# elastic-ai/elastic-gpu-agent

Hardware: AMD Instinct MI355X
Metric: fractional pods/GPU + p50 Allocate() RPC latency at 1/2/4/8 MI355X (higher is better)
Workload: dtype n/a; 1 GPU; model=gpushare-device-plugin, scenario=mixed, pods_per_gpu=16, backend=amdsmi, mem_unit_mib=1, global_batch=16, seq_len=0, parallelism=1 agent x 1 GPUs (1 load ranks)

## Files before the change

### elastic_gpu_agent_amd/isolation/__init__.py

```python
from __future__ import annotations

import json
import os
import threading
from typing import Dict, List, Optional, Tuple

from .. import consts
from ..types import GPUDevice
from .cumask import mask_hex, mask_words_from_cus, parse_mask_hex

try:
    from .._fastwire import atomic_write as _native_atomic_write
except ImportError:
    _native_atomic_write = None

AUX_MASK_PREFIX = "mask/"

_PRIORITY_RANK = {"low": 0, "normal": 1, "high": 2}


def priority_rank(priority: Optional[str]) -> int:
    return _PRIORITY_RANK.get(priority or "normal", 1)


class _Alloc:
    __slots__ = ("gpu", "cus", "rank", "orig_n_cus")

    def __init__(self, gpu: int, cus: set, rank: int, orig_n_cus: int):
        self.gpu = gpu
        self.cus = cus
        self.rank = rank
        self.orig_n_cus = orig_n_cus


class CUMaskAllocator:

    def __init__(self, storage, devices: List[GPUDevice], on_remask=None):
        self._storage = storage
        self._devices = {d.index: d for d in devices}
        self._lock = threading.Lock()
        self.on_remask = on_remask
        self._used: Dict[int, set] = {}
        self._by_hash: Dict[str, _Alloc] = {}
        for key, val in storage.aux_items(AUX_MASK_PREFIX):
            rec = json.loads(val)
            cus = self._mask_cus(rec["cu_mask"])
            gpu = rec.get("gpu_index")
            a = _Alloc(gpu, cus, priority_rank(rec.get("priority")),
                       rec.get("orig_cu_count", len(cus)))
            self._by_hash[key[len(AUX_MASK_PREFIX):]] = a
            self._used.setdefault(gpu, set()).update(cus)

    @staticmethod
    def _mask_cus(hexmask: str) -> set:
        cus = set()
        for w_i, w in enumerate(parse_mask_hex(hexmask)):
            for b in range(32):
                if w >> b & 1:
                    cus.add(w_i * 32 + b)
        return cus

    def _live_cus(self, gpu_index: int) -> set:
        return self._used.setdefault(gpu_index, set())

    def _free_pairs_by_xcd(self, gpu_index: int, total: int, xcds: int) -> List[List[int]]:
        per_xcd = total // xcds
# ... 11 lines not shown

    @staticmethod
    def _take_round_robin(free_by_xcd: List[List[int]], want: int,
                          taken: List[int]) -> None:
        while len(taken) < want and any(free_by_xcd):
            progress = False
            for free in free_by_xcd:
                if len(taken) >= want:
                    break
                if free:
                    taken.append(free.pop(0))
                    progress = True
            if not progress:
                break

    def _persist(self, alloc_hash: str, a: _Alloc, total: int, percent: int) -> Tuple[str, int]:
        cus = sorted(a.cus)
        words = mask_words_from_cus(cus, total)
        hexmask = mask_hex(words)
        rank_name = {0: "low", 1: "normal", 2: "high"}[a.rank]
        self._storage.aux_set(
            AUX_MASK_PREFIX + alloc_hash,
            json.dumps(
                {
                    "gpu_index": a.gpu,
                    "cu_mask": hexmask,
                    "cu_count": len(cus),
                    "percent": percent,
                    "priority": rank_name,
                    "orig_cu_count": a.orig_n_cus,
                }
            ),
        )
        return hexmask, len(cus)

    def _remask_victim(self, victim_hash: str, a: _Alloc, total: int) -> None:
        raw = self._storage.aux_get(AUX_MASK_PREFIX + victim_hash)
        percent = json.loads(raw).get("percent", 0) if raw else 0
        hexmask, n_cus = self._persist(victim_hash, a, total, percent)
        if self.on_remask is not None:
            try:
                self.on_remask(victim_hash, hexmask, n_cus)
            except Exception:
                pass

    def _reclaim_locked(self, gpu_index: int, need_pairs: int, my_rank: int,
                        total: int) -> List[int]:
        victims = sorted(
            (
# ... 50 lines not shown
            if want_pairs <= 0:
                continue
            free_by_xcd = self._free_pairs_by_xcd(gpu_index, total, xcds)
            taken: List[int] = []
            self._take_round_robin(free_by_xcd, want_pairs, taken)
            if not taken:
                return
            for cu0 in taken:
                a.cus.add(cu0)
                a.cus.add(cu0 + 1)
                used.add(cu0)
                used.add(cu0 + 1)
            self._remask_victim(h, a, total)

    def allocate(self, alloc_hash: str, gpu_index: int, percent: int,
                 priority: Optional[str] = None) -> Tuple[str, int]:
        dev = self._devices.get(gpu_index)
        total = dev.cu_count if dev else consts.GFX950_CU_COUNT
        xcds = dev.xcd_count if dev else consts.GFX950_XCD_COUNT
        per_xcd = total // xcds
        from .cumask import cu_count_for_percent

        n = cu_count_for_percent(percent, total)
        pairs_per_xcd = per_xcd // 2
        rank = priority_rank(priority)
        with self._lock:
            old = self._by_hash.pop(alloc_hash, None)
            if old is not None:
                still = set()
                for a in self._by_hash.values():
                    if a.gpu == old.gpu:
                        still |= a.cus
                self._used.setdefault(old.gpu, set()).difference_update(old.cus - still)
            used = self._live_cus(gpu_index)
            want = (n + 1) // 2
            taken: List[int] = []
            self._take_round_robin(
                self._free_pairs_by_xcd(gpu_index, total, xcds), want, taken)
            if len(taken) < want and rank > 0:
                taken.extend(self._reclaim_locked(
                    gpu_index, want - len(taken), rank, total))
            if len(taken) < want:
                pair_max_rank: Dict[int, int] = {}
                for a in self._by_hash.values():
                    if a.gpu != gpu_index:
                        continue
                    for cu in a.cus:
                        cu0 = cu - (cu % 2)
                        if a.rank > pair_max_rank.get(cu0, -1):
                            pair_max_rank[cu0] = a.rank
                candidates = []
                for p in range(pairs_per_xcd):
                    for xcd in range(xcds):
                        cu0 = xcd * per_xcd + 2 * p
                        if cu0 not in taken:
                            candidates.append(cu0)
                candidates.sort(key=lambda cu0: pair_max_rank.get(cu0, -1) > rank)
                taken.extend(candidates[: want - len(taken)])
            cus: List[int] = []
            for cu0 in taken[:want]:
                cus.extend((cu0, cu0 + 1))
            a = _Alloc(gpu_index, set(cus), rank, len(cus))
            hexmask, n_eff = self._persist(alloc_hash, a, total, percent)
            self._by_hash[alloc_hash] = a
            used.update(a.cus)
        return hexmask, n_eff

    def _release_cached(self, alloc_hash: str) -> Optional[int]:
        entry = self._by_hash.pop(alloc_hash, None)
        if entry is None:
            return None
        used = self._used.setdefault(entry.gpu, set())
        still = set()
        for a in self._by_hash.values():
            if a.gpu == entry.gpu:
                still |= a.cus
        used.difference_update(entry.cus - still)
        return entry.gpu

    def _dev_geometry(self, gpu_index: int) -> Tuple[int, int]:
        dev = self._devices.get(gpu_index)
        total = dev.cu_count if dev else consts.GFX950_CU_COUNT
        xcds = dev.xcd_count if dev else consts.GFX950_XCD_COUNT
        return total, xcds

    def release(self, alloc_hash: str) -> None:
        with self._lock:
            gpu = self._release_cached(alloc_hash)
            if gpu is not None:
                self._expand_shrunk_locked(gpu, *self._dev_geometry(gpu))
        self._storage.aux_delete(AUX_MASK_PREFIX + alloc_hash)

    def release_many(self, hashes) -> None:
        hashes = list(hashes)
        with self._lock:
            gpus = {self._release_cached(h) for h in hashes}
            for gpu in gpus:
                if gpu is not None:
                    self._expand_shrunk_locked(gpu, *self._dev_geometry(gpu))
        self._storage.aux_delete_many(AUX_MASK_PREFIX + h for h in hashes)

    def get(self, alloc_hash: str) -> Optional[dict]:
        raw = self._storage.aux_get(AUX_MASK_PREFIX + alloc_hash)
        return json.loads(raw) if raw else None


class _TxnAux:

    def __init__(self, conn):
        self._conn = conn

    def aux_items(self, prefix: str = "") -> list:
        return self._conn.execute(
            "SELECT key, val FROM aux WHERE key LIKE ?", (prefix + "%",)
# ... 46 lines not shown
    def _base(self):
        ver = self._aux.aux_get(self.VER_KEY)
        if self._cached_base is None or ver != self._cached_ver or ver is None:
            self._cached_base = CUMaskAllocator(self._aux, self._devices,
                                                on_remask=self.on_remask)
        return self._cached_base

    def _bump(self) -> None:
        import uuid

        self._cached_ver = uuid.uuid4().hex
        self._aux.aux_set(self.VER_KEY, self._cached_ver)

    def _txn(self):
        class _Txn:
            def __init__(s, conn):
                s.conn = conn

            def __enter__(s):
                import fcntl

                fcntl.flock(s.fd, fcntl.LOCK_EX)
                s.conn.execute("BEGIN IMMEDIATE")
                return s

            def __exit__(s, et, ev, tb):
                import fcntl

                try:
                    if et is None:
                        try:
                            s.conn.execute("COMMIT")
                        except Exception:
                            try:
                                s.conn.execute("ROLLBACK")
                            except Exception:
                                pass
                            raise
                    else:
                        try:
                            s.conn.execute("ROLLBACK")
                        except Exception:
                            pass
                finally:
                    fcntl.flock(s.fd, fcntl.LOCK_UN)
                return False

        t = _Txn(self._conn)
        t.fd = self._flock_fd
        return t

    def allocate(self, alloc_hash: str, gpu_index: int, percent: int,
                 priority: Optional[str] = None) -> Tuple[str, int]:
        with self._local, self._txn():
            out = self._base().allocate(alloc_hash, gpu_index, percent,
                                        priority=priority)
            self._bump()
            return out

    def release(self, alloc_hash: str) -> None:
        with self._local, self._txn():
            self._base().release(alloc_hash)
            self._bump()
# ... 113 lines not shown
```

### elastic_gpu_agent_amd/native/build.py

```python
from __future__ import annotations

import os
import subprocess
import sys
import sysconfig

ROCM = os.environ.get("ROCM_PATH", "/opt/rocm")
HERE = os.path.dirname(os.path.abspath(__file__))
PKG = os.path.dirname(HERE)
REPO = os.path.dirname(PKG)


def _run(cmd):
    print("+", " ".join(cmd), flush=True)
    subprocess.check_call(cmd)


def _newer(target: str, *sources: str) -> bool:
    if not os.path.exists(target):
        return False
    t = os.path.getmtime(target)
    return all(os.path.getmtime(s) <= t for s in sources)


# ... 10 lines not shown
    if not force and _newer(out, src):
        return out
    _run(
        ["g++", "-O2", "-std=c++17", "-shared", "-fPIC", src]
        + pybind_includes()
        + [f"-I{ROCM}/include", f"-L{ROCM}/lib", "-lamd_smi",
           f"-Wl,-rpath,{ROCM}/lib", "-o", out]
    )
    return out


def build_fastwire(force=False):
    src = os.path.join(HERE, "fastwire.cpp")
    ext = sysconfig.get_config_var("EXT_SUFFIX")
    out = os.path.join(PKG, f"_fastwire{ext}")
    headers = [os.path.join(HERE, h) for h in ("wirecore.h", "idruns.h", "hashmemo.h", "bindfx.h")]
    if not force and _newer(out, src, *headers):
        return out
    _run(
        ["g++", "-O2", "-std=c++17", "-shared", "-fPIC", src]
        + pybind_includes()
        + ["-o", out, "-lcrypto"]
    )
    return out


def build_etransport(force=False):
    src = os.path.join(HERE, "etransport.cpp")
    tables = os.path.join(HERE, "hpack_tables.h")
    gen = os.path.join(HERE, "gen_hpack_tables.py")
    if not os.path.exists(tables) or os.path.getmtime(tables) < os.path.getmtime(gen):
# ... 70 lines not shown
```

### elastic_gpu_agent_amd/native/build_fuzz.py

```python
from __future__ import annotations

import os
import subprocess
import sys

HERE = os.path.dirname(os.path.abspath(__file__))
REPO = os.path.dirname(os.path.dirname(HERE))
CLANGXX = os.environ.get(
    "EGPU_FUZZ_CLANGXX", "/opt/rocm/lib/llvm/bin/clang++")


def build(out=None):
    out = out or os.path.join(REPO, "bin", "egpu-fuzz")
    os.makedirs(os.path.dirname(out), exist_ok=True)
    cmd = [
        CLANGXX, "-O1", "-g", "-std=c++17",
        "-fsanitize=fuzzer,address",
        os.path.join(HERE, "fuzz_targets.cpp"),
        os.path.join(HERE, "devfilter.cpp"),
        "-I", HERE, "-o", out,
    ]
    print("+", " ".join(cmd), flush=True)
    subprocess.check_call(cmd)
    return out
# ... 60 lines not shown
def build_h2frame_selftest(out=None):
    out = out or os.path.join(REPO, "bin", "egpu-h2frame-selftest")
    return build_selftest(out, "h2frame_selftest.cpp")


def build_hash_memo_selftest(out=None):
    out = out or os.path.join(REPO, "bin", "egpu-hash-memo-selftest")
    return build_selftest(out, "hash_memo_selftest.cpp")


def build_bindfx_selftest(out=None):
    out = out or os.path.join(REPO, "bin", "egpu-bindfx-selftest")
    return build_selftest(out, "bindfx_selftest.cpp")


if __name__ == "__main__":
    if "--selftest" in sys.argv:
        rc = subprocess.call([build_selftest()])
        rc = rc or subprocess.call([build_stride_selftest()])
        rc = rc or subprocess.call([build_runs_selftest()])
        rc = rc or subprocess.call([build_ref_selftest()])
        rc = rc or subprocess.call([build_mx_ref_selftest()])
        rc = rc or subprocess.call([build_h2frame_selftest()])
        rc = rc or subprocess.call([build_hash_memo_selftest()])
        sys.exit(rc or subprocess.call([build_bindfx_selftest()]))
    binary = build()
    if "--replay" in sys.argv:
        sys.exit(replay(binary))
    if "--run" in sys.argv:
        secs = int(sys.argv[sys.argv.index("--run") + 1])
        sys.exit(run(binary, secs))
```

### elastic_gpu_agent_amd/native/fastwire.cpp

```cpp

#include <pybind11/pybind11.h>
#include <pybind11/stl.h>

#include <openssl/evp.h>

#include <algorithm>
#include <cerrno>
#include <cstdint>
#include <stdexcept>
#include <string>
#include <utility>
#include <vector>

#include "bindfx.h"
#include "wirecore.h"

namespace py = pybind11;

namespace {

using wirecore::DigestOut;
using wirecore::DigestScratch;
using wirecore::Reader;
using wirecore::ScratchGuard;
using wirecore::Span;
using wirecore::span_less;
using wirecore::spans_of;

py::list decode_string_list(py::bytes data) {
// ... 522 lines not shown
    bindfx::atomic_write(path, buf, (size_t)len);
  } catch (const bindfx::SysError& e) {
    raise_oserror(e);
  }
}

void unlink_many(const std::vector<std::string>& paths) {
  try {
    py::gil_scoped_release rel;
    bindfx::unlink_many(paths);
  } catch (const bindfx::SysError& e) {
    raise_oserror(e);
  }
}

}

PYBIND11_MODULE(_fastwire, m) {
  m.doc() = "wire-format accelerators for large fake-device ID sets";
  m.def("decode_string_list", &decode_string_list);
  m.def("decode_nested_string_lists", &decode_nested_string_lists);
  m.def("encode_device_list", &encode_device_list);
  m.def("encode_string_list", &encode_string_list);
  m.def("encode_nested_string_lists", &encode_nested_string_lists);
  m.def("encode_allocate_response", &encode_allocate_response);
  m.def("digest_allocate_request", &digest_allocate_request);
  m.def("decode_prestart_digest", &decode_prestart_digest);
  m.def("decode_prestart_digest2", &decode_prestart_digest2);
  m.def("decode_prestart_digest3", &decode_prestart_digest3);
  m.def("ids_to_runs", &ids_to_runs);
  m.def("expand_runs", &expand_runs);
  m.def("preferred_digest", &preferred_digest);
  m.def("podresources_digest", &podresources_digest);
  m.def("preferred_extract", &preferred_extract);
  m.def("hash_memo_configure", &hash_memo_configure, py::arg("entries"));
  m.def("hash_memo_stats", &hash_memo_stats);
  m.attr("HASH_MEMO_ENTRIES") = (long long)wirecore::kMemoEntries;
  m.attr("HASH_MEMO_MAX_KEY") = (long long)wirecore::kMemoMaxKey;
  m.def("make_links", &make_links, py::arg("pairs"));
  m.def("atomic_write", &atomic_write, py::arg("path"), py::arg("data"));
  m.def("unlink_many", &unlink_many, py::arg("paths"));
}
```

### elastic_gpu_agent_amd/plugins/gpushare.py

```python
from __future__ import annotations

import logging
import math
import threading
from typing import List

from .. import consts, topology
from ..kube.client import NotFound
from ..types import Device
from .config import GPUPluginConfig

log = logging.getLogger(__name__)


class GPUSharePluginBase:

    resource_name: str = ""

    def __init__(self, config: GPUPluginConfig):
        self.cfg = config
        self._devices_lock = threading.Lock()
        self._refresh = threading.Event()

    def fake_device_ids_for_gpu(self, gpu) -> List[str]:
# ... 211 lines not shown
            return self._fail(
                context, f"pod {pc.pod()} lacks {consts.ELASTIC_GPU_ASSUMED_ANNOTATION}=true"
            )
        raw = pod.container_gpu_indexes(pc.container)
        if raw is None:
            return self._fail(
                context,
                f"pod {pc.pod()} lacks annotation for container {pc.container}",
            )
        try:
            indexes = [int(x) for x in raw.split(",") if x != ""]
        except ValueError:
            return self._fail(context, f"bad GPU index annotation {raw!r}")
        created: List[str] = []
        try:
            self._bind(device, indexes, created, pod)
            pi = self.cfg.storage.load_or_create(pc.namespace, pc.name)
            pi.container_device_map[pc.container] = device
            self.cfg.storage.save(pi)
        except Exception as e:
            for alloc_id in created:
                self.cfg.operator.delete(-1, alloc_id)
            if self.cfg.cumask is not None:
                try:
                    self.cfg.cumask.release(device.hash)
                except Exception:
                    pass
            if self.cfg.limits is not None:
                self.cfg.limits.delete(device.hash)
            self._emit_event(pc, "EgpuBindFailed", f"bind {device.hash}: {e}")
            return self._fail(context, f"bind {device.hash}: {e}")
        return {}

    def _bind(self, device: Device, indexes: List[int], created: List[str],
# ... 60 lines not shown
        return resp

    def _bind(self, device: Device, indexes: List[int], created: List[str],
              pod=None):
        n_links = self.links_for(device.n_ids)
        if len(indexes) != n_links:
            raise ValueError(
                f"annotation has {len(indexes)} GPU indexes, expected {n_links}"
            )
        for i, idx in enumerate(indexes):
            alloc_id = f"{device.hash}-{i}"
            self.cfg.operator.create(idx, alloc_id)
            created.append(alloc_id)
        percent = device.n_ids
        priority = pod.qos_class() if pod is not None else None
        if percent < consts.GPU_PERCENT_EACH_CARD and self.cfg.cumask and self.cfg.limits:
            mask_hex, n_cus = self.cfg.cumask.allocate(
                device.hash, indexes[0], percent, priority=priority)
            self.cfg.limits.finalize(
                device.hash,
                gpu_indexes=indexes,
                devices=self.cfg.operator.devices(),
                cu_mask=mask_hex,
                cu_count=n_cus,
                priority=priority,
            )
        elif self.cfg.limits:
            self.cfg.limits.finalize(
                device.hash, gpu_indexes=indexes, devices=self.cfg.operator.devices(),
                priority=priority,
            )

    def _locator(self):
        return self.cfg.core_locator


class GPUShareMemoryPlugin(GPUSharePluginBase):

    resource_name = consts.RESOURCE_GPU_MEMORY

    def fake_device_ids_for_gpu(self, gpu) -> List[str]:
        unit = self.cfg.options.mem_unit_mib
        count = gpu.memory_mib // unit
        return [f"{gpu.index}-{slot:06d}" for slot in range(count)]

    def _allocate_one(self, alloc_hash: str, n_units: int) -> dict:
# ... 35 lines not shown
```

### elastic_gpu_agent_amd/storage/__init__.py

```python
from __future__ import annotations

import fcntl
import os
import sqlite3
import threading
from typing import Callable, Optional

from ..types import PodInfo


class NotFoundError(KeyError):
    pass


class Storage:

    def __init__(self, db_path: str, record_format: str = "runs"):
        if record_format not in ("runs", "list"):
            raise ValueError(f"record format {record_format!r}: want runs or list")
        self._record_format = record_format
        db_dir = os.path.dirname(os.path.abspath(db_path))
        os.makedirs(db_dir, exist_ok=True)
        self._path = db_path
        self._lock = threading.Lock()
# ... 102 lines not shown
        done.wait()
        if res:
            raise res[0]

    SUMMARY_PREFIX = "podsum/"

    @staticmethod
    def _summary(pod_info: PodInfo) -> str:
        import json as _json

        return _json.dumps({
            c: {"h": d.hash, "n": d.n_ids, "r": d.resource_name}
            for c, d in pod_info.container_device_map.items()
        }, separators=(",", ":"))

    def save(self, pod_info: PodInfo) -> None:
        self._submit([
            ("INSERT INTO pods(key, val) VALUES(?, ?) "
             "ON CONFLICT(key) DO UPDATE SET val=excluded.val",
             (pod_info.key(), pod_info.stored_val()
              if self._record_format == "runs" else pod_info.val())),
            ("INSERT INTO aux(key, val) VALUES(?, ?) "
             "ON CONFLICT(key) DO UPDATE SET val=excluded.val",
             (self.SUMMARY_PREFIX + pod_info.key(), self._summary(pod_info))),
        ])

    def rewrite_as_lists(self) -> int:
        with self._lock:
            rows = self._conn.execute(
                "SELECT key, val FROM pods WHERE instr(val, ?) > 0", (b'"Runs":',)
            ).fetchall()
        n = 0
        for key, val in rows:
            literal = PodInfo.from_raw(key, val).val()
            if literal != bytes(val):
                self._submit([("UPDATE pods SET val=? WHERE key=? AND val=?",
                               (literal, key, val))])
                n += 1
        return n

# ... 151 lines not shown
```

Measured before the change: 2918 pod-allocation-cycles/s.

## Move CU-mask occupancy to native bitset allocator and batch mask rows into pod save

Adds a C++ CUOccupancy class that tracks per-GPU CU occupancy as bitsets and handles placement, reclaim and release, used by default when _fastwire is built. The pure-Python set-based path is kept as a fallback. Mask rows can now be deferred and written in the same storage transaction as the pod record, which removes a separate aux write per allocation. The trade-off is a larger native surface, and the native policy has to match the Python placement semantics.

```diff
diff --git a/elastic_gpu_agent_amd/isolation/__init__.py b/elastic_gpu_agent_amd/isolation/__init__.py
--- a/elastic_gpu_agent_amd/isolation/__init__.py
+++ b/elastic_gpu_agent_amd/isolation/__init__.py
@@ -13,6 +13,11 @@
     from .._fastwire import atomic_write as _native_atomic_write
 except ImportError:
     _native_atomic_write = None
+
+try:
+    from .._fastwire import CUOccupancy as _NativeOccupancy
+except ImportError:
+    _NativeOccupancy = None
 
 AUX_MASK_PREFIX = "mask/"
 
@@ -35,21 +40,44 @@
 
 class CUMaskAllocator:
 
-    def __init__(self, storage, devices: List[GPUDevice], on_remask=None):
+    def __init__(self, storage, devices: List[GPUDevice], on_remask=None,
+                 policy: Optional[str] = None):
+        if policy not in (None, "native", "python"):
+            raise ValueError(f"policy {policy!r}: want native or python")
+        if policy == "native" and _NativeOccupancy is None:
+            raise RuntimeError("policy native: _fastwire is not built")
         self._storage = storage
         self._devices = {d.index: d for d in devices}
         self._lock = threading.Lock()
         self.on_remask = on_remask
+        self._occ = None
+        if policy != "python" and _NativeOccupancy is not None:
+            self._occ = _NativeOccupancy(consts.GFX950_CU_COUNT,
+                                         consts.GFX950_XCD_COUNT)
+            for d in devices:
+                self._occ.set_geometry(d.index, d.cu_count, d.xcd_count)
         self._used: Dict[int, set] = {}
         self._by_hash: Dict[str, _Alloc] = {}
         for key, val in storage.aux_items(AUX_MASK_PREFIX):
             rec = json.loads(val)
+            if self._occ is not None:
+                words = [w & 0xFFFFFFFF for w in parse_mask_hex(rec["cu_mask"])]
+                self._occ.load(
+                    key[len(AUX_MASK_PREFIX):], rec.get("gpu_index"), words,
+                    priority_rank(rec.get("priority")),
+                    rec.get("orig_cu_count", sum(bin(w).count("1") for w in words)),
+                    rec.get("percent", 0))
+                continue
             cus = self._mask_cus(rec["cu_mask"])
             gpu = rec.get("gpu_index")
             a = _Alloc(gpu, cus, priority_rank(rec.get("priority")),
                        rec.get("orig_cu_count", len(cus)))
             self._by_hash[key[len(AUX_MASK_PREFIX):]] = a
             self._used.setdefault(gpu, set()).update(cus)
+
+    @property
+    def storage(self):
+        return self._storage
 
     @staticmethod
     def _mask_cus(hexmask: str) -> set:
@@ -91,25 +119,37 @@
             if not progress:
                 break
 
-    def _persist(self, alloc_hash: str, a: _Alloc, total: int, percent: int) -> Tuple[str, int]:
+    @staticmethod
+    def _row(gpu, hexmask: str, n_cus: int, percent: int, rank: int,
+             orig_n_cus: int) -> str:
+        return json.dumps(
+            {
+                "gpu_index": gpu,
+                "cu_mask": hexmask,
+                "cu_count": n_cus,
+                "percent": percent,
+                "priority": {0: "low", 1: "normal", 2: "high"}[rank],
+                "orig_cu_count": orig_n_cus,
+            }
+        )
+
+    def _persist(self, alloc_hash: str, a: _Alloc, total: int, percent: int,
+                 deferred: Optional[list] = None) -> Tuple[str, int]:
         cus = sorted(a.cus)
         words = mask_words_from_cus(cus, total)
         hexmask = mask_hex(words)
-        rank_name = {0: "low", 1: "normal", 2: "high"}[a.rank]
-        self._storage.aux_set(
+        self._aux_set(
             AUX_MASK_PREFIX + alloc_hash,
-            json.dumps(
-                {
-                    "gpu_index": a.gpu,
-                    "cu_mask": hexmask,
-                    "cu_count": len(cus),
-                    "percent": percent,
-                    "priority": rank_name,
-                    "orig_cu_count": a.orig_n_cus,
-                }
-            ),
+            self._row(a.gpu, hexmask, len(cus), percent, a.rank, a.orig_n_cus),
+            deferred,
         )
         return hexmask, len(cus)
+
+    def _aux_set(self, key: str, val: str, deferred: Optional[list]) -> None:
+        if deferred is not None:
+            deferred.append((key, val))
+        else:
+            self._storage.aux_set(key, val)
 
     def _remask_victim(self, victim_hash: str, a: _Alloc, total: int) -> None:
         raw = self._storage.aux_get(AUX_MASK_PREFIX + victim_hash)
@@ -190,56 +230,95 @@
             self._remask_victim(h, a, total)
 
     def allocate(self, alloc_hash: str, gpu_index: int, percent: int,
-                 priority: Optional[str] = None) -> Tuple[str, int]:
-        dev = self._devices.get(gpu_index)
-        total = dev.cu_count if dev else consts.GFX950_CU_COUNT
-        xcds = dev.xcd_count if dev else consts.GFX950_XCD_COUNT
+                 priority: Optional[str] = None, defer: bool = False):
+        total, xcds = self._dev_geometry(gpu_index)
+        from .cumask import cu_count_for_percent
+
+        n = cu_count_for_percent(percent, total)
+        rank = priority_rank(priority)
+        rows: Optional[list] = [] if defer else None
+        with self._lock:
+            place = (self._allocate_native_locked if self._occ is not None
+                     else self._allocate_python_locked)
+            hexmask, n_eff = place(alloc_hash, gpu_index, percent, n, rank,
+                                   total, xcds, rows)
+        return (hexmask, n_eff, rows) if defer else (hexmask, n_eff)
+
+    def _allocate_native_locked(self, alloc_hash: str, gpu_index: int, percent: int,
+                                n: int, rank: int, total: int, xcds: int,
+                                deferred: Optional[list]) -> Tuple[str, int]:
+        words, n_eff, orig_n_cus, victims = self._occ.allocate(
+            alloc_hash, gpu_index, n, rank, percent, total, xcds)
+        try:
+            self._remask_native(victims)
+            return self._persist_native(
+                (alloc_hash, words, n_eff, percent, gpu_index, rank, orig_n_cus),
+                deferred)
+        except BaseException:
+            self._occ.drop(alloc_hash)
+            raise
+
+    def _persist_native(self, row, deferred: Optional[list] = None) -> Tuple[str, int]:
+        alloc_hash, words, n_cus, percent, gpu, rank, orig_n_cus = row
+        hexmask = mask_hex(words)
+        self._aux_set(AUX_MASK_PREFIX + alloc_hash,
+                      self._row(gpu, hexmask, n_cus, percent, rank, orig_n_cus),
+                      deferred)
+        return hexmask, n_cus
+
+    def _remask_native(self, rows) -> None:
+        for row in rows:
+            hexmask, n_cus = self._persist_native(row)
+            if self.on_remask is not None:
+                try:
+                    self.on_remask(row[0], hexmask, n_cus)
+                except Exception:
+                    pass
+
+    def _allocate_python_locked(self, alloc_hash: str, gpu_index: int, percent: int,
+                                n: int, rank: int, total: int, xcds: int,
+                                deferred: Optional[list]) -> Tuple[str, int]:
         per_xcd = total // xcds
-        from .cumask import cu_count_for_percent
-
-        n = cu_count_for_percent(percent, total)
         pairs_per_xcd = per_xcd // 2
-        rank = priority_rank(priority)
-        with self._lock:
-            old = self._by_hash.pop(alloc_hash, None)
-            if old is not None:
-                still = set()
-                for a in self._by_hash.values():
-                    if a.gpu == old.gpu:
-                        still |= a.cus
-                self._used.setdefault(old.gpu, set()).difference_update(old.cus - still)
-            used = self._live_cus(gpu_index)
-            want = (n + 1) // 2
-            taken: List[int] = []
-            self._take_round_robin(
-                self._free_pairs_by_xcd(gpu_index, total, xcds), want, taken)
-            if len(taken) < want and rank > 0:
-                taken.extend(self._reclaim_locked(
-                    gpu_index, want - len(taken), rank, total))
-            if len(taken) < want:
-                pair_max_rank: Dict[int, int] = {}
-                for a in self._by_hash.values():
-                    if a.gpu != gpu_index:
-                        continue
-                    for cu in a.cus:
-                        cu0 = cu - (cu % 2)
-                        if a.rank > pair_max_rank.get(cu0, -1):
-                            pair_max_rank[cu0] = a.rank
-                candidates = []
-                for p in range(pairs_per_xcd):
-                    for xcd in range(xcds):
-                        cu0 = xcd * per_xcd + 2 * p
-                        if cu0 not in taken:
-                            candidates.append(cu0)
-                candidates.sort(key=lambda cu0: pair_max_rank.get(cu0, -1) > rank)
-                taken.extend(candidates[: want - len(taken)])
-            cus: List[int] = []
-            for cu0 in taken[:want]:
-                cus.extend((cu0, cu0 + 1))
-            a = _Alloc(gpu_index, set(cus), rank, len(cus))
-            hexmask, n_eff = self._persist(alloc_hash, a, total, percent)
-            self._by_hash[alloc_hash] = a
-            used.update(a.cus)
+        old = self._by_hash.pop(alloc_hash, None)
+        if old is not None:
+            still = set()
+            for a in self._by_hash.values():
+                if a.gpu == old.gpu:
+                    still |= a.cus
+            self._used.setdefault(old.gpu, set()).difference_update(old.cus - still)
+        used = self._live_cus(gpu_index)
+        want = (n + 1) // 2
+        taken: List[int] = []
+        self._take_round_robin(
+            self._free_pairs_by_xcd(gpu_index, total, xcds), want, taken)
+        if len(taken) < want and rank > 0:
+            taken.extend(self._reclaim_locked(
+                gpu_index, want - len(taken), rank, total))
+        if len(taken) < want:
+            pair_max_rank: Dict[int, int] = {}
+            for a in self._by_hash.values():
+                if a.gpu != gpu_index:
+                    continue
+                for cu in a.cus:
+                    cu0 = cu - (cu % 2)
+                    if a.rank > pair_max_rank.get(cu0, -1):
+                        pair_max_rank[cu0] = a.rank
+            candidates = []
+            for p in range(pairs_per_xcd):
+                for xcd in range(xcds):
+                    cu0 = xcd * per_xcd + 2 * p
+                    if cu0 not in taken:
+                        candidates.append(cu0)
+            candidates.sort(key=lambda cu0: pair_max_rank.get(cu0, -1) > rank)
+            taken.extend(candidates[: want - len(taken)])
+        cus: List[int] = []
+        for cu0 in taken[:want]:
+            cus.extend((cu0, cu0 + 1))
+        a = _Alloc(gpu_index, set(cus), rank, len(cus))
+        hexmask, n_eff = self._persist(alloc_hash, a, total, percent, deferred)
+        self._by_hash[alloc_hash] = a
+        used.update(a.cus)
         return hexmask, n_eff
 
     def _release_cached(self, alloc_hash: str) -> Optional[int]:
@@ -262,18 +341,24 @@
 
     def release(self, alloc_hash: str) -> None:
         with self._lock:
-            gpu = self._release_cached(alloc_hash)
-            if gpu is not None:
-                self._expand_shrunk_locked(gpu, *self._dev_geometry(gpu))
+            if self._occ is not None:
+                self._remask_native(self._occ.release(alloc_hash))
+            else:
+                gpu = self._release_cached(alloc_hash)
+                if gpu is not None:
+                    self._expand_shrunk_locked(gpu, *self._dev_geometry(gpu))
         self._storage.aux_delete(AUX_MASK_PREFIX + alloc_hash)
 
     def release_many(self, hashes) -> None:
         hashes = list(hashes)
         with self._lock:
-            gpus = {self._release_cached(h) for h in hashes}
-            for gpu in gpus:
-                if gpu is not None:
-                    self._expand_shrunk_locked(gpu, *self._dev_geometry(gpu))
+            if self._occ is not None:
+                self._remask_native(self._occ.release_many(hashes))
+            else:
+                gpus = dict.fromkeys(self._release_cached(h) for h in hashes)
+                for gpu in gpus:
+                    if gpu is not None:
+                        self._expand_shrunk_locked(gpu, *self._dev_geometry(gpu))
         self._storage.aux_delete_many(AUX_MASK_PREFIX + h for h in hashes)
 
     def get(self, alloc_hash: str) -> Optional[dict]:
@@ -350,8 +435,9 @@
 
     def _txn(self):
         class _Txn:
-            def __init__(s, conn):
+            def __init__(s, conn, owner):
                 s.conn = conn
+                s.owner = owner
 
             def __enter__(s):
                 import fcntl
@@ -368,12 +454,14 @@
                         try:
                             s.conn.execute("COMMIT")
                         except Exception:
+                            s.owner._cached_base = None
                             try:
                                 s.conn.execute("ROLLBACK")
                             except Exception:
                                 pass
                             raise
                     else:
+                        s.owner._cached_base = None
                         try:
                             s.conn.execute("ROLLBACK")
                         except Exception:
@@ -382,7 +470,7 @@
                     fcntl.flock(s.fd, fcntl.LOCK_UN)
                 return False
 
-        t = _Txn(self._conn)
+        t = _Txn(self._conn, self)
         t.fd = self._flock_fd
         return t
 
diff --git a/elastic_gpu_agent_amd/native/build.py b/elastic_gpu_agent_amd/native/build.py
--- a/elastic_gpu_agent_amd/native/build.py
+++ b/elastic_gpu_agent_amd/native/build.py
@@ -48,7 +48,8 @@
     src = os.path.join(HERE, "fastwire.cpp")
     ext = sysconfig.get_config_var("EXT_SUFFIX")
     out = os.path.join(PKG, f"_fastwire{ext}")
-    headers = [os.path.join(HERE, h) for h in ("wirecore.h", "idruns.h", "hashmemo.h", "bindfx.h")]
+    headers = [os.path.join(HERE, h) for h in ("wirecore.h", "idruns.h", "hashmemo.h", "bindfx.h",
+                                                   "cuocc.h")]
     if not force and _newer(out, src, *headers):
         return out
     _run(
diff --git a/elastic_gpu_agent_amd/native/build_fuzz.py b/elastic_gpu_agent_amd/native/build_fuzz.py
--- a/elastic_gpu_agent_amd/native/build_fuzz.py
+++ b/elastic_gpu_agent_amd/native/build_fuzz.py
@@ -98,6 +98,11 @@
     return build_selftest(out, "bindfx_selftest.cpp")
 
 
+def build_cuocc_selftest(out=None):
+    out = out or os.path.join(REPO, "bin", "egpu-cuocc-selftest")
+    return build_selftest(out, "cuocc_selftest.cpp")
+
+
 if __name__ == "__main__":
     if "--selftest" in sys.argv:
         rc = subprocess.call([build_selftest()])
@@ -107,7 +112,8 @@
         rc = rc or subprocess.call([build_mx_ref_selftest()])
         rc = rc or subprocess.call([build_h2frame_selftest()])
         rc = rc or subprocess.call([build_hash_memo_selftest()])
-        sys.exit(rc or subprocess.call([build_bindfx_selftest()]))
+        rc = rc or subprocess.call([build_bindfx_selftest()])
+        sys.exit(rc or subprocess.call([build_cuocc_selftest()]))
     binary = build()
     if "--replay" in sys.argv:
         sys.exit(replay(binary))
diff --git a/elastic_gpu_agent_amd/native/cuocc.h b/elastic_gpu_agent_amd/native/cuocc.h
--- /dev/null
+++ b/elastic_gpu_agent_amd/native/cuocc.h
@@ -0,0 +1,351 @@
+#pragma once
+
+#include <algorithm>
+#include <cstddef>
+#include <cstdint>
+#include <iterator>
+#include <limits>
+#include <list>
+#include <optional>
+#include <stdexcept>
+#include <string>
+#include <unordered_map>
+#include <utility>
+#include <vector>
+
+namespace cuocc {
+
+constexpr int64_t kNoGpu = std::numeric_limits<int64_t>::min();
+
+class Bits {
+ public:
+  bool test(int64_t i) const {
+    if (i < 0) return false;
+    size_t k = (size_t)i >> 6;
+    return k < w_.size() && (w_[k] >> (i & 63) & 1);
+  }
+  void set(int64_t i) {
+    if (i < 0) return;
+    size_t k = (size_t)i >> 6;
+    if (k >= w_.size()) w_.resize(k + 1, 0);
+    w_[k] |= uint64_t(1) << (i & 63);
+  }
+  void clear(int64_t i) {
+    if (i < 0) return;
+    size_t k = (size_t)i >> 6;
+    if (k < w_.size()) w_[k] &= ~(uint64_t(1) << (i & 63));
+  }
+  void merge(const Bits& o) {
+    if (o.w_.size() > w_.size()) w_.resize(o.w_.size(), 0);
+    for (size_t k = 0; k < o.w_.size(); ++k) w_[k] |= o.w_[k];
+  }
+  int64_t count() const {
+    int64_t n = 0;
+    for (uint64_t w : w_) n += __builtin_popcountll(w);
+    return n;
+  }
+  int64_t top() const {
+    for (size_t k = w_.size(); k-- > 0;)
+      if (w_[k]) return (int64_t)(k * 64 + 63 - __builtin_clzll(w_[k]));
+    return -1;
+  }
+  template <class F>
+  void for_each(F f) const {
+    for (size_t k = 0; k < w_.size(); ++k)
+      for (uint64_t w = w_[k]; w; w &= w - 1)
+        f((int64_t)(k * 64 + __builtin_ctzll(w)));
+  }
+
+ private:
+  std::vector<uint64_t> w_;
+};
+
+struct Row {
+  std::string hash;
+  int64_t gpu = 0;
+  std::vector<uint32_t> words;
+  int64_t n_cus = 0;
+  int rank = 0;
+  int64_t orig_n_cus = 0;
+  int64_t percent = 0;
+};
+
+struct Placement {
+  Row own;
+  std::vector<Row> victims;
+};
+
+class Occupancy {
+ public:
+  Occupancy(int64_t default_total, int64_t default_xcds)
+      : default_geo_{default_total, default_xcds} {
+    check_geometry(default_total, default_xcds);
+  }
+
+  void set_geometry(int64_t gpu, int64_t total, int64_t xcds) {
+    check_geometry(total, xcds);
+    geo_[gpu] = Geometry{total, xcds};
+  }
+
+  size_t size() const { return order_.size(); }
+
+  void load(const std::string& hash, int64_t gpu, const std::vector<uint32_t>& words,
+            int rank, int64_t orig_n_cus, int64_t percent) {
+    Alloc a;
+    a.hash = hash;
+    a.gpu = gpu;
+    for (size_t i = 0; i < words.size(); ++i)
+      for (uint32_t w = words[i]; w; w &= w - 1)
+        a.cus.set((int64_t)(i * 32 + __builtin_ctz(w)));
+    a.rank = rank;
+    a.orig_n_cus = orig_n_cus;
+    a.percent = percent;
+    auto it = index_.find(hash);
+    if (it != index_.end()) {
+      *it->second = std::move(a);
+      return;
+    }
+    order_.push_back(std::move(a));
+    index_.emplace(hash, std::prev(order_.end()));
+  }
+
+  Placement allocate(const std::string& hash, int64_t gpu, int64_t n_cus, int rank,
+                     int64_t percent, int64_t total, int64_t xcds) {
+    check_geometry(total, xcds);
+    if (n_cus < 0) throw std::invalid_argument("cuocc: negative CU count");
+    drop(hash);
+    Placement out;
+    const int64_t want = (n_cus + 1) / 2;
+    std::vector<int64_t> taken;
+    {
+      FreePairs free = free_pairs(gpu, total, xcds);
+      take_round_robin(free, want, taken);
+    }
+    if ((int64_t)taken.size() < want && rank > 0)
+      reclaim(gpu, want - (int64_t)taken.size(), rank, total, taken, out.victims);
+    if ((int64_t)taken.size() < want) overlap(gpu, want, rank, total, xcds, taken);
+    if ((int64_t)taken.size() > want) taken.resize((size_t)want);
+    Alloc a;
+    a.hash = hash;
+    a.gpu = gpu;
+    for (int64_t cu0 : taken) {
+      a.cus.set(cu0);
+      a.cus.set(cu0 + 1);
+    }
+    a.rank = rank;
+    a.orig_n_cus = 2 * (int64_t)taken.size();
+    a.percent = percent;
+    out.own = row_of(a, total);
+    order_.push_back(std::move(a));
+    index_.emplace(hash, std::prev(order_.end()));
+    return out;
+  }
+
+  std::optional<int64_t> drop(const std::string& hash) {
+    auto it = index_.find(hash);
+    if (it == index_.end()) return std::nullopt;
+    int64_t gpu = it->second->gpu;
+    order_.erase(it->second);
+    index_.erase(it);
+    return gpu;
+  }
+
+  std::vector<Row> release(const std::string& hash) {
+    std::vector<Row> grown;
+    std::optional<int64_t> gpu = drop(hash);
+    if (gpu && *gpu != kNoGpu) expand(*gpu, grown);
+    return grown;
+  }
+
+  std::vector<Row> release_many(const std::vector<std::string>& hashes) {
+    std::vector<int64_t> gpus;
+    for (const std::string& h : hashes) {
+      std::optional<int64_t> gpu = drop(h);
+      if (gpu && *gpu != kNoGpu && std::find(gpus.begin(), gpus.end(), *gpu) == gpus.end())
+        gpus.push_back(*gpu);
+    }
+    std::vector<Row> grown;
+    for (int64_t gpu : gpus) expand(gpu, grown);
+    return grown;
+  }
+
+  std::optional<Row> get(const std::string& hash, int64_t total) const {
+    auto it = index_.find(hash);
+    if (it == index_.end()) return std::nullopt;
+    return row_of(*it->second, total);
+  }
+
+ private:
+  struct Alloc {
+    std::string hash;
+    int64_t gpu = 0;
+    Bits cus;
+    int rank = 0;
+    int64_t orig_n_cus = 0;
+    int64_t percent = 0;
+  };
+  struct Geometry {
+    int64_t total, xcds;
+  };
+  struct FreePairs {
+    std::vector<std::vector<int64_t>> by_xcd;
+    std::vector<size_t> next;
+  };
+
+  static void check_geometry(int64_t total, int64_t xcds) {
+    if (xcds < 1) throw std::invalid_argument("cuocc: XCD count below 1");
+    if (total < 0) throw std::invalid_argument("cuocc: negative CU total");
+  }
+
+  Geometry geometry(int64_t gpu) const {
+    auto it = geo_.find(gpu);
+    return it == geo_.end() ? default_geo_ : it->second;
+  }
+
+  static Row row_of(const Alloc& a, int64_t total) {
+    Row r;
+    r.hash = a.hash;
+    r.gpu = a.gpu;
+    size_t n_words = (size_t)((total + 31) / 32);
+    int64_t top = a.cus.top();
+    if (top >= 0) n_words = std::max(n_words, (size_t)(top / 32 + 1));
+    r.words.assign(n_words, 0);
+    a.cus.for_each([&](int64_t cu) { r.words[(size_t)(cu / 32)] |= uint32_t(1) << (cu % 32); });
+    r.n_cus = a.cus.count();
+    r.rank = a.rank;
+    r.orig_n_cus = a.orig_n_cus;
+    r.percent = a.percent;
+    return r;
+  }
+
+  Bits used(int64_t gpu) const {
+    Bits u;
+    for (const Alloc& a : order_)
+      if (a.gpu == gpu) u.merge(a.cus);
+    return u;
+  }
+
+  FreePairs free_pairs(int64_t gpu, int64_t total, int64_t xcds) const {
+    const int64_t per_xcd = total / xcds, pairs_per_xcd = per_xcd / 2;
+    const Bits u = used(gpu);
+    FreePairs f;
+    f.by_xcd.resize((size_t)xcds);
+    f.next.assign((size_t)xcds, 0);
+    for (int64_t x = 0; x < xcds; ++x)
+      for (int64_t p = 0; p < pairs_per_xcd; ++p) {
+        int64_t cu0 = x * per_xcd + 2 * p;
+        if (!u.test(cu0) && !u.test(cu0 + 1)) f.by_xcd[(size_t)x].push_back(cu0);
+      }
+    return f;
+  }
+
+  static void take_round_robin(FreePairs& f, int64_t want, std::vector<int64_t>& taken) {
+    bool progress = true;
+    while ((int64_t)taken.size() < want && progress) {
+      progress = false;
+      for (size_t x = 0; x < f.by_xcd.size(); ++x) {
+        if ((int64_t)taken.size() >= want) break;
+        if (f.next[x] < f.by_xcd[x].size()) {
+          taken.push_back(f.by_xcd[x][f.next[x]++]);
+          progress = true;
+        }
+      }
+    }
+  }
+
+  void reclaim(int64_t gpu, int64_t need, int my_rank, int64_t total,
+               std::vector<int64_t>& taken, std::vector<Row>& changed_rows) {
+    struct Victim {
+      Alloc* a;
+      int64_t n;
+    };
+    std::vector<Victim> victims;
+    for (Alloc& a : order_) {
+      int64_t n = a.cus.count();
+      if (a.gpu == gpu && a.rank < my_rank && n > 2) victims.push_back({&a, n});
+    }
+    std::stable_sort(victims.begin(), victims.end(), [](const Victim& l, const Victim& r) {
+      return l.a->rank != r.a->rank ? l.a->rank < r.a->rank : l.n > r.n;
+    });
+    std::vector<int64_t> freed;
+    std::vector<Alloc*> changed;
+    for (const Victim& v : victims) {
+      if ((int64_t)freed.size() >= need) break;
+      std::vector<int64_t> pairs;
+      v.a->cus.for_each([&](int64_t cu) {
+        int64_t cu0 = cu - cu % 2;
+        if (pairs.empty() || pairs.back() != cu0) pairs.push_back(cu0);
+      });
+      int64_t give = std::min((int64_t)pairs.size() - 1, need - (int64_t)freed.size());
+      if (give <= 0) continue;
+      for (size_t i = pairs.size() - (size_t)give; i < pairs.size(); ++i) {
+        v.a->cus.clear(pairs[i]);
+        v.a->cus.clear(pairs[i] + 1);
+        freed.push_back(pairs[i]);
+      }
+      changed.push_back(v.a);
+    }
+    if (freed.empty()) return;
+    for (Alloc* a : changed) changed_rows.push_back(row_of(*a, total));
+    const Bits still = used(gpu);
+    for (int64_t cu0 : freed)
+      if (!still.test(cu0) && !still.test(cu0 + 1)) taken.push_back(cu0);
+  }
+
+  void overlap(int64_t gpu, int64_t want, int rank, int64_t total, int64_t xcds,
+               std::vector<int64_t>& taken) const {
+    const int64_t per_xcd = total / xcds, pairs_per_xcd = per_xcd / 2;
+    std::vector<int> pair_max_rank((size_t)(total / 2 + 1), -1);
+    for (const Alloc& a : order_) {
+      if (a.gpu != gpu) continue;
+      a.cus.for_each([&](int64_t cu) {
+        size_t p = (size_t)(cu / 2);
+        if (p < pair_max_rank.size() && a.rank > pair_max_rank[p]) pair_max_rank[p] = a.rank;
+      });
+    }
+    Bits have;
+    for (int64_t cu0 : taken) have.set(cu0);
+    std::vector<int64_t> mine, above;
+    for (int64_t p = 0; p < pairs_per_xcd; ++p)
+      for (int64_t x = 0; x < xcds; ++x) {
+        int64_t cu0 = x * per_xcd + 2 * p;
+        if (have.test(cu0)) continue;
+        int held = cu0 % 2 ? -1 : pair_max_rank[(size_t)(cu0 / 2)];
+        (held > rank ? above : mine).push_back(cu0);
+      }
+    for (const std::vector<int64_t>* cands : {&mine, &above})
+      for (int64_t cu0 : *cands) {
+        if ((int64_t)taken.size() >= want) return;
+        taken.push_back(cu0);
+      }
+  }
+
+  void expand(int64_t gpu, std::vector<Row>& grown) {
+    const Geometry g = geometry(gpu);
+    std::vector<Alloc*> shrunk;
+    for (Alloc& a : order_)
+      if (a.gpu == gpu && a.cus.count() < a.orig_n_cus) shrunk.push_back(&a);
+    std::stable_sort(shrunk.begin(), shrunk.end(),
+                     [](const Alloc* l, const Alloc* r) { return l->rank > r->rank; });
+    for (Alloc* a : shrunk) {
+      int64_t want = (a->orig_n_cus - a->cus.count()) / 2;
+      if (want <= 0) continue;
+      FreePairs free = free_pairs(gpu, g.total, g.xcds);
+      std::vector<int64_t> taken;
+      take_round_robin(free, want, taken);
+      if (taken.empty()) return;
+      for (int64_t cu0 : taken) {
+        a->cus.set(cu0);
+        a->cus.set(cu0 + 1);
+      }
+      grown.push_back(row_of(*a, g.total));
+    }
+  }
+
+  Geometry default_geo_;
+  std::unordered_map<int64_t, Geometry> geo_;
+  std::list<Alloc> order_;
+  std::unordered_map<std::string, std::list<Alloc>::iterator> index_;
+};
+
+}
diff --git a/elastic_gpu_agent_amd/native/cuocc_selftest.cpp b/elastic_gpu_agent_amd/native/cuocc_selftest.cpp
--- /dev/null
+++ b/elastic_gpu_agent_amd/native/cuocc_selftest.cpp
@@ -0,0 +1,254 @@
+#include <cstdint>
+#include <cstdio>
+#include <map>
+#include <string>
+#include <vector>
+
+#include "cuocc.h"
+
+namespace {
+
+int failures = 0;
+
+#define CHECK(cond, what)                                                       \
+  do {                                                                          \
+    if (!(cond)) {                                                              \
+      fprintf(stderr, "FAIL %s:%d %s (%s)\n", __FILE__, __LINE__, #cond, what); \
+      ++failures;                                                               \
+    }                                                                           \
+  } while (0)
+
+using cuocc::Occupancy;
+using cuocc::Placement;
+using cuocc::Row;
+
+std::string hex(const std::vector<uint32_t>& words) {
+  std::string out;
+  char b[16];
+  for (size_t i = 0; i < words.size(); ++i) {
+    snprintf(b, sizeof b, "%s%08x", i ? "," : "", words[i]);
+    out += b;
+  }
+  return out;
+}
+
+int64_t popcount(const std::vector<uint32_t>& words) {
+  int64_t n = 0;
+  for (uint32_t w : words) n += __builtin_popcount(w);
+  return n;
+}
+
+std::string brief(const std::vector<Row>& rows) {
+  std::string out;
+  for (const Row& r : rows) out += r.hash + ":" + hex(r.words) + ":" + std::to_string(r.n_cus) + " ";
+  return out;
+}
+
+int64_t cus_for(int64_t percent, int64_t total) {
+  if (percent >= 100) return total;
+  int64_t n = std::max<int64_t>(1, (percent * total + 50) / 100);
+  return std::min(total, n + (n & 1));
+}
+
+void fixed_cases() {
+  {
+    Occupancy o(32, 1);
+    Placement lo = o.allocate("lo", 0, cus_for(75, 32), 0, 75, 32, 1);
+    CHECK(hex(lo.own.words) == "00ffffff" && lo.own.n_cus == 24 && lo.victims.empty(), "lo");
+    Placement hi = o.allocate("hi", 0, cus_for(75, 32), 2, 75, 32, 1);
+    CHECK(hex(hi.own.words) == "ffffff00" && hi.own.n_cus == 24, "hi");
+    CHECK(brief(hi.victims) == "lo:000000ff:8 ", brief(hi.victims).c_str());
+    CHECK(hi.victims.size() == 1 && hi.victims[0].percent == 75 && hi.victims[0].orig_n_cus == 24,
+          "the victim keeps its percent and its original size");
+    std::vector<Row> grown = o.release("hi");
+    CHECK(brief(grown) == "lo:00ffffff:24 ", brief(grown).c_str());
+  }
+  {
+    Occupancy o(8, 2);
+    CHECK(hex(o.allocate("a", 0, 4, 1, 50, 8, 2).own.words) == "00000033", "a");
+    CHECK(hex(o.allocate("b", 0, 4, 1, 50, 8, 2).own.words) == "000000cc", "b");
+    CHECK(hex(o.allocate("c", 0, 4, 0, 50, 8, 2).own.words) == "00000033", "c overlaps a");
+    Placement d = o.allocate("d", 0, 6, 2, 75, 8, 2);
+    CHECK(hex(d.own.words) == "000000f0" && d.own.n_cus == 4 && d.own.orig_n_cus == 6,
+          "d counts the pair it was given twice");
+    CHECK(brief(d.victims) == "c:00000003:2 a:00000003:2 b:0000000c:2 ", brief(d.victims).c_str());
+    CHECK(o.release("a").empty(), "nothing free after a alone leaves");
+    std::vector<Row> grown = o.release("d");
+    CHECK(brief(grown) == "b:0000003c:4 c:000000c3:4 ", brief(grown).c_str());
+  }
+  {
+    Occupancy o(36, 4);
+    CHECK(hex(o.allocate("a", 0, 22, 0, 60, 36, 4).own.words) == "78fc7e3f,00000000", "a");
+    CHECK(hex(o.allocate("b", 0, 22, 0, 60, 36, 4).own.words) == "9b0d9ecf,00000007", "b");
+    Placement c = o.allocate("c", 0, 12, 1, 30, 36, 4);
+    CHECK(hex(c.own.words) == "18fc0603,00000000" && c.own.n_cus == 12, hex(c.own.words).c_str());
+    CHECK(brief(c.victims) == "a:00007e3f,00000000:12 ", brief(c.victims).c_str());
+  }
+  {
+    for (int reallocate = 0; reallocate < 2; ++reallocate) {
+      Occupancy o(32, 1);
+      o.allocate("A", 0, 12, 0, 37, 32, 1);
+      o.allocate("B", 0, 12, 0, 37, 32, 1);
+      if (reallocate) {
+        Placement again = o.allocate("A", 0, 12, 0, 37, 32, 1);
+        CHECK(hex(again.own.words) == "00000fff", "A keeps its CUs, not its place");
+      }
+      Placement h = o.allocate("H", 0, 16, 2, 50, 32, 1);
+      CHECK(h.victims.size() == 1 && h.victims[0].hash == (reallocate ? "B" : "A"),
+            brief(h.victims).c_str());
+    }
+  }
+  {
+    Occupancy o(256, 8);
+    CHECK(o.release("nobody").empty() && o.release_many({"x", "y", "x"}).empty(), "unknown");
+    o.load("nogpu", cuocc::kNoGpu, {0xf}, 0, 4, 5);
+    Placement p = o.allocate("p", 0, 256, 2, 99, 256, 8);
+    CHECK(p.own.n_cus == 256 && p.victims.empty(), "a row without a GPU is in nobody's way");
+    CHECK(o.release("nogpu").empty() && o.size() == 1, "and its release expands nobody");
+    CHECK(!o.drop("nogpu") && o.drop("p") && o.size() == 0, "drop");
+    bool threw = false;
+    try {
+      o.allocate("z", 0, 2, 1, 1, 256, 0);
+    } catch (const std::invalid_argument&) {
+      threw = true;
+    }
+    CHECK(threw && o.size() == 0, "zero XCDs");
+  }
+  {
+    Occupancy o(8, 2);
+    std::vector<uint32_t> wide(40, 0);
+    wide[0] = 0x3;
+    wide[39] = 0xff00;
+    o.load("wide", 0, wide, 0, 10, 50);
+    Placement hi = o.allocate("hi", 0, 8, 2, 99, 8, 2);
+    CHECK(hi.own.words.size() == 40 && hi.own.words[39] == 0xc000 && hi.own.words[0] == 0xfc,
+          hex(hi.own.words).c_str());
+    CHECK(hi.victims.size() == 1 && hi.victims[0].words.size() == 40 &&
+              hi.victims[0].words[39] == 0x3f00 && hi.victims[0].n_cus == 8,
+          brief(hi.victims).c_str());
+    std::vector<Row> grown = o.release("hi");
+    CHECK(grown.size() == 1 && grown[0].words[0] == 0xf && grown[0].n_cus == 10, brief(grown).c_str());
+  }
+}
+
+struct Rng {
+  uint64_t state;
+  uint64_t operator()() {
+    state ^= state << 13;
+    state ^= state >> 7;
+    state ^= state << 17;
+    return state;
+  }
+  int64_t below(int64_t n) { return (int64_t)((*this)() % (uint64_t)n); }
+};
+
+struct Geo {
+  int64_t total, xcds;
+};
+
+void check_row(const Row& r, int64_t total, const char* what) {
+  CHECK((int64_t)r.words.size() >= (total + 31) / 32, what);
+  CHECK(popcount(r.words) == r.n_cus, what);
+  CHECK(r.n_cus <= r.orig_n_cus || r.orig_n_cus < 0, what);
+}
+
+void random_sequences(const std::vector<Geo>& gpus, uint64_t seed) {
+  Rng rng{seed};
+  Occupancy o(256, 8);
+  for (size_t g = 0; g < gpus.size(); ++g) o.set_geometry((int64_t)g, gpus[g].total, gpus[g].xcds);
+  std::vector<uint32_t> wide((size_t)(gpus[0].total + 31) / 32 + 3, 0);
+  wide[0] = 0x3;
+  wide.back() = 0xf0;
+  o.load("wide", 0, wide, 0, 12, 7);
+  o.load("nogpu", cuocc::kNoGpu, {0xffff, 0, 0xf}, 1, 20, 5);
+  std::vector<uint32_t> spill((size_t)(gpus[0].total + 31) / 32, 0);
+  spill.back() = 0xf0000000u;
+  o.load("spill", 0, spill, 0, 8, 9);
+
+  std::vector<std::string> names = {"wide", "nogpu", "spill"};
+  for (int i = 0; i < 12; ++i) names.push_back("h" + std::to_string(i));
+  std::map<std::string, int> rank_of = {{"wide", 0}, {"nogpu", 1}, {"spill", 0}};
+  for (int step = 0; step < 600; ++step) {
+    int64_t roll = rng.below(100);
+    const std::string& name = names[(size_t)rng.below((int64_t)names.size())];
+    if (roll < 55) {
+      int64_t gpu = rng.below((int64_t)gpus.size());
+      const Geo& geo = gpus[(size_t)gpu];
+      int rank = (int)rng.below(3);
+      int64_t percent = 1 + rng.below(99);
+      int64_t n = cus_for(percent, geo.total);
+      size_t before = o.size();
+      bool live = o.get(name, geo.total).has_value();
+      Placement p = o.allocate(name, gpu, n, rank, percent, geo.total, geo.xcds);
+      rank_of[name] = rank;
+      CHECK(o.size() == before + (live ? 0 : 1), "one more allocation, or the same one again");
+      check_row(p.own, geo.total, "own row");
+      CHECK(p.own.gpu == gpu && p.own.rank == rank && p.own.percent == percent, "own row");
+      CHECK(p.own.orig_n_cus <= 2 * ((n + 1) / 2) && p.own.n_cus >= 2, "size");
+      CHECK(rank > 0 || p.victims.empty(), "rank 0 reclaims from nobody");
+      for (const Row& v : p.victims) {
+        check_row(v, geo.total, "victim row");
+        CHECK(v.gpu == gpu && v.rank < rank && v.n_cus >= 1 && v.n_cus < v.orig_n_cus, "victim");
+        CHECK(rank_of[v.hash] == v.rank, "victim rank");
+        std::optional<Row> now = o.get(v.hash, geo.total);
+        CHECK(now && now->words == v.words, "the victim's row is what the occupancy holds");
+      }
+      std::optional<Row> mine = o.get(name, geo.total);
+      CHECK(mine && mine->words == p.own.words && mine->orig_n_cus == p.own.orig_n_cus, "get");
+    } else if (roll < 80) {
+      size_t before = o.size();
+      bool live = o.get(name, 0).has_value();
+      std::vector<Row> grown = o.release(name);
+      CHECK(o.size() == before - (live ? 1 : 0), "release");
+      CHECK(live || grown.empty(), "an unknown hash expands nobody");
+      for (const Row& r : grown) check_row(r, gpus[(size_t)r.gpu].total, "grown row");
+    } else if (roll < 93) {
+      std::vector<std::string> batch;
+      for (int64_t k = rng.below(6); k > 0; --k) batch.push_back(names[(size_t)rng.below((int64_t)names.size())]);
+      batch.push_back("never-allocated");
+      for (const Row& r : o.release_many(batch)) {
+        check_row(r, gpus[(size_t)r.gpu].total, "grown row");
+        CHECK(r.n_cus <= r.orig_n_cus, "grows back no further than its original size");
+      }
+    } else {
+      CHECK(o.release("unknown" + std::to_string(rng.below(3))).empty(), "unknown hash");
+    }
+  }
+  names.push_back("never-allocated");
+  o.release_many(names);
+  CHECK(o.size() == 0, "everything released");
+  for (size_t g = 0; g < gpus.size(); ++g) {
+    const Geo& geo = gpus[g];
+    std::vector<uint32_t> seen((size_t)(geo.total + 31) / 32, 0);
+    int64_t pairs = (geo.total / geo.xcds / 2) * geo.xcds, held = 0;
+    for (int i = 0; held < pairs; ++i) {
+      int64_t n = 2 * (1 + rng.below(3));
+      if (held + n / 2 > pairs) n = 2 * (pairs - held);
+      Placement p = o.allocate("fill" + std::to_string(g) + "-" + std::to_string(i), (int64_t)g, n, 1,
+                               1, geo.total, geo.xcds);
+      CHECK(p.own.n_cus == n && p.own.words.size() == seen.size(), "fills exactly");
+      for (size_t w = 0; w < seen.size() && w < p.own.words.size(); ++w) {
+        CHECK((seen[w] & p.own.words[w]) == 0, "disjoint while there is room");
+        seen[w] |= p.own.words[w];
+      }
+      held += n / 2;
+    }
+  }
+}
+
+}
+
+int main() {
+  fixed_cases();
+  const std::vector<std::vector<Geo>> geometries = {
+      {{8, 2}}, {{32, 1}}, {{36, 4}}, {{304, 8}}, {{256, 8}}, {{256, 8}, {36, 4}}};
+  uint64_t seed = 0x9e3779b97f4a7c15ull;
+  for (const auto& gpus : geometries)
+    for (int round = 0; round < 3; ++round) random_sequences(gpus, seed += 0x632be59bd9b4e019ull);
+  if (failures) {
+    fprintf(stderr, "cuocc selftest: %d failure(s)\n", failures);
+    return 1;
+  }
+  printf("cuocc selftest: ok\n");
+  return 0;
+}
diff --git a/elastic_gpu_agent_amd/native/fastwire.cpp b/elastic_gpu_agent_amd/native/fastwire.cpp
--- a/elastic_gpu_agent_amd/native/fastwire.cpp
+++ b/elastic_gpu_agent_amd/native/fastwire.cpp
@@ -13,6 +13,7 @@
 #include <vector>
 
 #include "bindfx.h"
+#include "cuocc.h"
 #include "wirecore.h"
 
 namespace py = pybind11;
@@ -565,6 +566,63 @@
   }
 }
 
+
+py::tuple cuocc_row(const cuocc::Row& r) {
+  py::object gpu = r.gpu == cuocc::kNoGpu ? py::object(py::none()) : py::object(py::int_(r.gpu));
+  return py::make_tuple(r.hash, r.words, r.n_cus, r.percent, gpu, r.rank, r.orig_n_cus);
+}
+
+py::list cuocc_rows(const std::vector<cuocc::Row>& rows) {
+  py::list out;
+  for (const cuocc::Row& r : rows) out.append(cuocc_row(r));
+  return out;
+}
+
+int64_t cuocc_gpu(const py::object& gpu) {
+  return gpu.is_none() ? cuocc::kNoGpu : gpu.cast<int64_t>();
+}
+
+void bind_cuocc(py::module_& m) {
+  py::class_<cuocc::Occupancy>(m, "CUOccupancy")
+      .def(py::init<int64_t, int64_t>(), py::arg("default_total"), py::arg("default_xcds"))
+      .def("set_geometry", &cuocc::Occupancy::set_geometry, py::arg("gpu"), py::arg("total"),
+           py::arg("xcds"))
+      .def("__len__", &cuocc::Occupancy::size)
+      .def("load",
+           [](cuocc::Occupancy& o, const std::string& hash, const py::object& gpu,
+              const std::vector<uint32_t>& words, int rank, int64_t orig_n_cus, int64_t percent) {
+             o.load(hash, cuocc_gpu(gpu), words, rank, orig_n_cus, percent);
+           },
+           py::arg("hash"), py::arg("gpu"), py::arg("words"), py::arg("rank"),
+           py::arg("orig_n_cus"), py::arg("percent"))
+      .def("allocate",
+           [](cuocc::Occupancy& o, const std::string& hash, int64_t gpu, int64_t n_cus, int rank,
+              int64_t percent, int64_t total, int64_t xcds) {
+             cuocc::Placement p = o.allocate(hash, gpu, n_cus, rank, percent, total, xcds);
+             return py::make_tuple(p.own.words, p.own.n_cus, p.own.orig_n_cus,
+                                   cuocc_rows(p.victims));
+           },
+           py::arg("hash"), py::arg("gpu"), py::arg("n_cus"), py::arg("rank"),
+           py::arg("percent"), py::arg("total"), py::arg("xcds"))
+      .def("drop",
+           [](cuocc::Occupancy& o, const std::string& hash) { return o.drop(hash).has_value(); },
+           py::arg("hash"))
+      .def("release",
+           [](cuocc::Occupancy& o, const std::string& hash) { return cuocc_rows(o.release(hash)); },
+           py::arg("hash"))
+      .def("release_many",
+           [](cuocc::Occupancy& o, const std::vector<std::string>& hashes) {
+             return cuocc_rows(o.release_many(hashes));
+           },
+           py::arg("hashes"))
+      .def("get",
+           [](const cuocc::Occupancy& o, const std::string& hash, int64_t total) -> py::object {
+             std::optional<cuocc::Row> r = o.get(hash, total);
+             return r ? py::object(cuocc_row(*r)) : py::object(py::none());
+           },
+           py::arg("hash"), py::arg("total"));
+}
+
 }
 
 PYBIND11_MODULE(_fastwire, m) {
@@ -591,4 +649,5 @@
   m.def("make_links", &make_links, py::arg("pairs"));
   m.def("atomic_write", &atomic_write, py::arg("path"), py::arg("data"));
   m.def("unlink_many", &unlink_many, py::arg("paths"));
-}
+  bind_cuocc(m);
+}
diff --git a/elastic_gpu_agent_amd/plugins/gpushare.py b/elastic_gpu_agent_amd/plugins/gpushare.py
--- a/elastic_gpu_agent_amd/plugins/gpushare.py
+++ b/elastic_gpu_agent_amd/plugins/gpushare.py
@@ -249,10 +249,13 @@
             return self._fail(context, f"bad GPU index annotation {raw!r}")
         created: List[str] = []
         try:
-            self._bind(device, indexes, created, pod)
+            aux_rows = self._bind(device, indexes, created, pod)
             pi = self.cfg.storage.load_or_create(pc.namespace, pc.name)
             pi.container_device_map[pc.container] = device
-            self.cfg.storage.save(pi)
+            if aux_rows is not None:
+                self.cfg.storage.save_with_aux(pi, aux_rows)
+            else:
+                self.cfg.storage.save(pi)
         except Exception as e:
             for alloc_id in created:
                 self.cfg.operator.delete(-1, alloc_id)
@@ -343,9 +346,14 @@
             created.append(alloc_id)
         percent = device.n_ids
         priority = pod.qos_class() if pod is not None else None
+        aux_rows = None
         if percent < consts.GPU_PERCENT_EACH_CARD and self.cfg.cumask and self.cfg.limits:
-            mask_hex, n_cus = self.cfg.cumask.allocate(
-                device.hash, indexes[0], percent, priority=priority)
+            if self._mask_rows_ride_the_save():
+                mask_hex, n_cus, aux_rows = self.cfg.cumask.allocate(
+                    device.hash, indexes[0], percent, priority=priority, defer=True)
+            else:
+                mask_hex, n_cus = self.cfg.cumask.allocate(
+                    device.hash, indexes[0], percent, priority=priority)
             self.cfg.limits.finalize(
                 device.hash,
                 gpu_indexes=indexes,
@@ -359,6 +367,16 @@
                 device.hash, gpu_indexes=indexes, devices=self.cfg.operator.devices(),
                 priority=priority,
             )
+        return aux_rows
+
+    def _mask_rows_ride_the_save(self) -> bool:
+        from ..isolation import CUMaskAllocator
+
+        cumask, storage = self.cfg.cumask, self.cfg.storage
+        return (isinstance(cumask, CUMaskAllocator)
+                and storage is not None
+                and cumask.storage is storage
+                and hasattr(storage, "save_with_aux"))
 
     def _locator(self):
         return self.cfg.core_locator
diff --git a/elastic_gpu_agent_amd/storage/__init__.py b/elastic_gpu_agent_amd/storage/__init__.py
--- a/elastic_gpu_agent_amd/storage/__init__.py
+++ b/elastic_gpu_agent_amd/storage/__init__.py
@@ -140,8 +140,18 @@
             for c, d in pod_info.container_device_map.items()
         }, separators=(",", ":"))
 
-    def save(self, pod_info: PodInfo) -> None:
+    def save(self, pod_info: PodInfo, aux_rows=()) -> None:
         self._submit([
+            ("INSERT INTO aux(key, val) VALUES(?, ?) "
+             "ON CONFLICT(key) DO UPDATE SET val=excluded.val", (key, val))
+            for key, val in aux_rows
+        ] + self._save_ops(pod_info))
+
+    def save_with_aux(self, pod_info: PodInfo, aux_rows) -> None:
+        self.save(pod_info, aux_rows)
+
+    def _save_ops(self, pod_info: PodInfo) -> list:
+        return [
             ("INSERT INTO pods(key, val) VALUES(?, ?) "
              "ON CONFLICT(key) DO UPDATE SET val=excluded.val",
              (pod_info.key(), pod_info.stored_val()
@@ -149,7 +159,7 @@
             ("INSERT INTO aux(key, val) VALUES(?, ?) "
              "ON CONFLICT(key) DO UPDATE SET val=excluded.val",
              (self.SUMMARY_PREFIX + pod_info.key(), self._summary(pod_info))),
-        ])
+        ]
 
     def rewrite_as_lists(self) -> int:
         with self._lock:
```

After: 3296 pod-allocation-cycles/s, median of 5. 13.0% higher.
